# HKU-BAL/Clair

Hardware: AMD Instinct MI355X
Metric: candidate sites/sec (whole node) (higher is better)
Workload: dtype f32 (matmuls as 2-way fp16 split on MFMA with fp32 accumulate; gates/activations fp32); 1 GPU; ONT 122HD34 weights-shape model (random init), synthetic ont-profile pileup tensors, batch=1024, 4 batches in flight per GPU, inputs resident in HBM; batch=1024, streams=4, candidates_total=38912, device_warm_steps=251, collective=none (1 rank), transport=none

## Files before the change

### clair_amd/_capi.py

```python
import ctypes
import os

import numpy as np

from clair_amd._hostapi import Handle

_HERE = os.path.dirname(os.path.abspath(__file__))
LIB_PATH = os.environ.get("CLAIR_AMD_LIB") or os.path.join(_HERE, "libclair_amd.so")

c_int, c_i64, c_vp, c_cp, c_dbl = ctypes.c_int, ctypes.c_int64, ctypes.c_void_p, ctypes.c_char_p, ctypes.c_double
p_vp, p_i64 = ctypes.POINTER(c_vp), ctypes.POINTER(c_i64)


def _sig(*argtypes, **kw):
    return kw.get("restype", c_int), list(argtypes)


_SUBMIT_EX = (c_vp, c_int, c_vp, c_int, c_i64, c_int, c_vp, c_vp, c_vp, c_vp, c_vp, c_vp)
_INFLATE_BLOCKS = (c_vp, c_vp, c_i64, c_int, c_vp, c_vp, c_vp, c_vp, c_vp, c_vp)
SIGNATURES = {
    "clair_abi_version": _sig(),
    "clair_device_count": _sig(),
    "clair_device_pci_bus_id": _sig(c_int, c_cp, c_int),
    "clair_last_error": _sig(c_vp, restype=c_cp),
# ... 380 lines not shown
        mask = int(bool(on))
        if only:
            mask = 0
            for k in only:
                mask |= 1 << KERNEL_NAMES.index(k)
        self._check(self._lib.clair_timing_enable(self._h, mask), "clair_timing_enable")

    def timing_reset(self):
        self._check(self._lib.clair_timing_reset(self._h), "clair_timing_reset")

    def kernel_times(self):
        ms = np.zeros(len(KERNEL_NAMES), dtype=np.float64)
        cnt = np.zeros(len(KERNEL_NAMES), dtype=np.int64)
        self._check(self._lib.clair_kernel_times(self._h, _ptr(ms), _ptr(cnt)), "clair_kernel_times")
        return {k: (float(ms[i]), int(cnt[i])) for i, k in enumerate(KERNEL_NAMES)}

    def kernel_workgroups(self, n):
        wg = np.zeros(len(KERNEL_NAMES), dtype=np.int32)
        self._check(self._lib.clair_kernel_workgroups(self._h, int(n), _ptr(wg)), "clair_kernel_workgroups")
        return {k: int(wg[i]) for i, k in enumerate(KERNEL_NAMES)}

    def counter(self, name):
        v = ctypes.c_int64()
        self._check(self._lib.clair_engine_counter(self._h, ("fused_launches", "fused_recoveries").index(name), ctypes.byref(v)), "clair_engine_counter")
        return int(v.value)

    def debug_read(self, slot, which, shape):
        out = np.empty(shape, dtype=np.float32)
        self._check(self._lib.clair_debug_read(self._h, int(slot), int(which), _ptr(out), out.size), "clair_debug_read")
        return out


class SiteTable(DeviceHandle):

    def __init__(self, engine):
        self._lib = engine._lib
        self._engine = engine
        out = self._own(self._lib.clair_sites_destroy, self._lib.clair_last_error)
        engine._check(self._lib.clair_sites_create(engine._h, out), "clair_sites_create")
        self.n_out = 0

    def _check(self, rc, what):
        if rc != 0:
            raise EngineError("%s failed: %s" % (what, self._last_error(self._engine._h).decode()))

    def begin_source(self, positions):
        p = np.ascontiguousarray(positions, dtype=np.int64)
# ... 390 lines not shown
```

### clair_amd/_hostapi.py

```python
import ctypes
import os

import numpy as np

_HERE = os.path.dirname(os.path.abspath(__file__))
LIB_PATH = os.path.join(_HERE, "libclair_host.so")
vp, cp, i32, i64, f64 = ctypes.c_void_p, ctypes.c_char_p, ctypes.c_int, ctypes.c_int64, ctypes.c_double
p_vp, p_i32, p_i64 = ctypes.POINTER(vp), ctypes.POINTER(i32), ctypes.POINTER(i64)


def _sig(*argtypes, **kw):
    return kw.get("restype", i32), list(argtypes)


_DECODE_ROWS = (vp, vp, vp, vp, vp, cp, vp, i32, i32, i32, i32, i32, i32, vp, i64, p_i64, p_i32)
_FEED = (vp, vp, i64, i32, p_i64)
SIGNATURES = {
    "clair_host_abi_version": _sig(),
    "clair_host_last_error": _sig(restype=cp),
    "clair_host_threads": _sig(i32),
    "clair_host_crc32c": _sig(cp, i64, restype=ctypes.c_uint32),
    "clair_host_counts_to_input_i16": _sig(vp, i64, vp),
    "clair_host_counts_to_input_i32": _sig(vp, i64, vp),
    "clair_host_parse_tensors": _sig(vp, i64, i32, i32, vp, vp, p_i32, p_i32, p_i64),
# ... 41 lines not shown
    "clair_host_bam_render": _sig(vp, vp, vp, i64, i32, i64, i64, p_vp, p_i64),
    "clair_host_faidx": _sig(cp, cp, i64, i64, vp, i64, p_i64),
    "clair_host_bam_set_inflater": _sig(vp, vp, vp, i32),
    "clair_host_inflate_block": _sig(vp, i64, vp, i64, p_i64, ctypes.POINTER(ctypes.c_uint32), p_i32),
    "clair_host_inflate_bgzf": _sig(vp, i64, vp, p_i64, p_i32),
    "clair_host_ensemble_average": _sig(vp, i32, i64, vp),
    "clair_host_ensemble_quantise": _sig(vp, i64, vp),
    "clair_host_ensemble_value": _sig(vp, i64, vp),
    "clair_host_overlap_keep": _sig(vp, i64, vp),
    "clair_host_train_set_key": _sig(cp, i64, i32, p_i64),
    "clair_host_train_set_sample": _sig(vp, i64, vp, i64, f64, f64, i64, vp, vp, vp, p_i64, p_i64),
    "clair_host_train_set_pair_count": _sig(vp, i64, vp, i64, vp, vp, i64, p_i64, p_i64),
    "clair_host_train_set_ratio": _sig(i64, f64, i64, ctypes.POINTER(f64)),
    "clair_host_train_set_pair_keep": _sig(vp, i64, vp, i64, vp, vp, i64, f64, i64, vp, p_i64, p_i64),
    "clair_host_train_set_labels": _sig(vp, vp, i64, vp, vp, i64, vp, vp, i64, vp, vp),
    "clair_host_sites_create": _sig(p_vp),
    "clair_host_sites_destroy": _sig(vp, restype=None),
    "clair_host_sites_begin_source": _sig(vp, vp, i64, p_i64),
    "clair_host_sites_add_rows": _sig(vp, i64, vp, i64, vp, vp, vp),
    "clair_host_sites_finish": _sig(vp, i32, i32, p_i64),
    "clair_host_sites_info": _sig(vp, i64, i64, vp, vp, vp),
    "clair_host_sites_rows": _sig(vp, i64, i64, vp),
    "clair_host_sites_windows": _sig(vp, i64, i64, vp),
}
SYMBOLS = tuple(SIGNATURES)
N_VALUES = 1056
_lib = None


def load():
    global _lib
    if _lib is None:
        if not os.path.isfile(LIB_PATH):
            raise RuntimeError("%s not found: run `python -m clair_amd.build`" % LIB_PATH)
        lib = ctypes.CDLL(LIB_PATH)
        for name, (restype, argtypes) in SIGNATURES.items():
            fn = getattr(lib, name)
            fn.restype, fn.argtypes = restype, argtypes
        if lib.clair_host_abi_version() != 6:
            raise RuntimeError("libclair_host.so has ABI version %d, expected 6: run `python -m clair_amd.build`"
                               % lib.clair_host_abi_version())
        _lib = lib
    return _lib


class Handle(object):
# ... 774 lines not shown
    kv, kn = ctypes.c_int64(0), ctypes.c_int64(0)
    _ts_check(load().clair_host_train_set_pair_keep(p.ctypes.data, len(p), t.ctypes.data, len(t), bs.ctypes.data, be.ctypes.data, nb, float(r), int(key),
                                                    kept.ctypes.data, ctypes.byref(kv), ctypes.byref(kn)))
    return kept[:kv.value + kn.value], kv.value


def train_set_pair(centres, truth, bed, amp, key):
    v, c = train_set_pair_count(centres, truth, bed)
    r = train_set_ratio(v, amp, c)
    kept, kv = train_set_pair_keep(centres, truth, bed, r, key)
    return kept, dict(v=v, c=c, r=r, kept_var=kv, kept_non=len(kept) - kv)


def train_set_labels(centres, centre_base, truth, truth_labels, bed):
    p = np.ascontiguousarray(centres, dtype=np.int64)
    b = np.ascontiguousarray(centre_base, dtype=np.uint8)
    t = np.ascontiguousarray(truth, dtype=np.int64)
    tl = np.ascontiguousarray(truth_labels, dtype=np.uint8).reshape(len(t), 4)
    bs, be, nb = merged_bed(bed)
    labels, in_set = np.zeros((len(p), 4), np.uint8), np.zeros(len(p), np.uint8)
    _ts_check(load().clair_host_train_set_labels(p.ctypes.data, b.ctypes.data, len(p), t.ctypes.data, tl.ctypes.data, len(t), bs.ctypes.data, be.ctypes.data, nb,
                                                 labels.ctypes.data, in_set.ctypes.data))
    return labels, in_set
```

### clair_amd/build.py

```python
import os
import subprocess
import sys

HERE = os.path.dirname(os.path.abspath(__file__))
SRCS = [os.path.join(HERE, "csrc", f) for f in ("engine.hip", "comm.hip", "frontend.hip", "inflate.hip", "overlap.hip", "train.hip")]
OUT = os.path.join(HERE, "libclair_amd.so")
HIPCC = os.environ.get("HIPCC", "/opt/rocm/bin/hipcc")


def csrc_digest(root=None):
    import hashlib
    root = root or os.path.join(HERE, "csrc")
    h = hashlib.sha256()
    for f in sorted(os.listdir(root)):
        if (f.endswith(".hip.h") and not f.startswith("train_")) or f in ("engine.hip", "weight_images.h", "device_buffer.h", "ensemble_core.h"):
            h.update(f.encode() + b"\0" + open(os.path.join(root, f), "rb").read() + b"\0")
    return h.hexdigest()[:16]


def needs_build():
    if not os.path.isfile(OUT):
        return True
    newest = max(os.path.getmtime(os.path.join(dp, f))
                 for dp, _, fs in os.walk(os.path.join(HERE, "csrc")) for f in fs)
    newest = max([newest] + [os.path.getmtime(os.path.join(HERE, "..", "include", h)) for h in ("clair_amd.h", "clair_call.h", "clair_reads.h")])
    return newest > os.path.getmtime(OUT)


HOST_SRCS = [os.path.join(HERE, "hostsrc", f) for f in ("host_io.cpp", "host_decode.cpp", "host_pileup.cpp", "host_sampack.cpp",
                                                              "host_bam.cpp", "host_inflate.cpp", "host_indel.cpp", "host_ensemble.cpp", "host_overlap.cpp", "host_sites.cpp", "host_train_set.cpp")]
HOST_OUT = os.path.join(HERE, "libclair_host.so")
CXX = os.environ.get("CXX", "g++")


def build_host(force=False):
    hdrs = [os.path.join(HERE, "..", "include", h) for h in ("clair_host.h", "clair_reads.h", "clair_call.h", "clair_amd.h")]
    hdrs.append(os.path.join(HERE, "hostsrc", "sam_line.h"))
    hdrs.append(os.path.join(HERE, "csrc", "inflate_core.h"))
    hdrs.append(os.path.join(HERE, "csrc", "indel_lookup_core.h"))
    hdrs.append(os.path.join(HERE, "csrc", "ensemble_core.h"))
    hdrs.append(os.path.join(HERE, "csrc", "overlap_core.h"))
    hdrs.append(os.path.join(HERE, "csrc", "train_set_core.h"))
    if (force or not os.path.isfile(HOST_OUT)
            or max([os.path.getmtime(f) for f in HOST_SRCS + hdrs]) > os.path.getmtime(HOST_OUT)):
        subprocess.check_call([CXX, "-O3", "-std=c++17", "-ffp-contract=off", "-pthread", "-shared", "-fPIC", "-Wall"] + HOST_SRCS + ["-o", HOST_OUT, "-lz"])
    return HOST_OUT


def build(force=False, verbose=False):
    build_host(force)
    if not force and not needs_build():
        return OUT
    cmd = [HIPCC, "--offload-arch=gfx950", "-O3", "-fno-slp-vectorize", "-std=c++17", "-shared", "-fPIC"] + SRCS + ["-o", OUT, "-ldl"]
    if verbose:
        cmd.insert(1, "-Rpass-analysis=kernel-resource-usage")
    subprocess.check_call(cmd)
    return OUT


WAITALL_OUT = os.path.join(HERE, "libclair_amd_waitall.so")


def build_waitall():
    subprocess.check_call([HIPCC, "--offload-arch=gfx950", "-O3", "-fno-slp-vectorize", "-std=c++17", "-shared", "-fPIC", "-DCLAIR_WAIT_ALL"]
                          + SRCS + ["-o", WAITALL_OUT, "-ldl"])
# ... 20 lines not shown
```

### clair_amd/csrc/engine.hip

```cpp
#include "../../include/clair_amd.h"

#include <hip/hip_runtime.h>
#include <ctype.h>

#include <algorithm>
#include <atomic>
#include <cmath>
#include <cstdarg>
#include <cstdio>
#include <cstdlib>
#include <condition_variable>
#include <cstring>
#include <deque>
#include <list>
#include <memory>
#include <mutex>
#include <string>
#include <thread>
#include <vector>

#include "common.hip.h"
#include "dense.hip.h"
#include "decode.hip.h"
#include "evaluate.hip.h"
#include "ensemble.hip.h"
#include "gemm_split.hip.h"
#include "lstm32.hip.h"
#include "lstm32_pair.hip.h"
#include "lstm2_fused.hip.h"
#include "sites.hip.h"
#include "device_buffer.h"
#include "weight_images.h"

using namespace clair;

namespace {

thread_local std::string g_create_error;
thread_local std::string *g_error_sink = nullptr;

constexpr LayerSizes LAYER_SIZES = {T_POS, F_IN, HID, L3_UNITS, L4_UNITS, L5_UNITS, L34_GROUPS, L34_KS, L34_CH, L32_X_SHIFT};

struct TimedLaunch {
    int kernel;
    hipEvent_t start, stop;
};

struct Lane {
    hipStream_t stream = nullptr;
    DeviceBuffer zx;
    DeviceBuffer a1;
    DeviceBuffer a2;
    DeviceBuffer l4part;
    DeviceBuffer fuse_flags;
    unsigned fuse_ticket = 0;
    int last_n_pad = 0;
    std::mutex order;
    std::vector<TimedLaunch> timed;
    std::vector<hipEvent_t> free_events;
    struct FusedRun { const float *x; float *out; int n; int slot; };
    std::vector<FusedRun> fused_runs;
};

struct Slot {
    int lane = 0;
    hipStream_t cin = nullptr, cout = nullptr;
    hipEvent_t ev_in = nullptr, ev_done = nullptr, ev_out = nullptr;
    DeviceBuffer d_x;
    DeviceBuffer d_out;
    PinnedBuffer h_out;
    PinnedBuffer h_x;
    DeviceBuffer d_counts;
    DeviceBuffer d_records;
    PinnedBuffer h_counts;
    DeviceBuffer d_centre; PinnedBuffer h_centre;
    DeviceBuffer d_calls; PinnedBuffer h_calls;
    clair_call_t *o_calls = nullptr;
    DeviceBuffer d_labels; PinnedBuffer h_labels;
    DeviceBuffer d_acc;
    DeviceBuffer d_seq; PinnedBuffer h_seq;
    float *o_gt21 = nullptr, *o_gt = nullptr, *o_l1 = nullptr, *o_l2 = nullptr;
    int pending_n = 0;
    bool refetch = false;
    int staged = 0;
    std::string worker_error;
};

struct ModelWeights {
// ... 20 lines not shown
    int cur = 0;
    int64_t src_n = -1;
    DeviceBuffer pos, lb, is_new, before, row_of;
    DeviceBuffer overflow;
    bool finished = false;
    int64_t n_out = 0;
    DeviceBuffer keep, out_before, out_row, out_key, out_count, out_seq, avg;
    DeviceBuffer gathered;
    SiteRows rows() const { return SiteRows{key.as<int64_t>(), count.as<int>(), acc.as<double>(), x.as<float>(), centre.as<unsigned char>(), seq.as<unsigned char>()}; }
};

struct clair_engine {
    int device = 0;
    int max_batch = 0;
    int max_pad = 0;
    unsigned timing_mask = 0;
    int lstm2_pair = -1;
    std::atomic<int> lstm2_fused{0};
    int fused_groups = 4;
    int64_t fused_launches = 0;
    int64_t fused_fault_at = 0;
    int fused_recoveries = 0;
    int proj2_groups = 8;
    bool l34_stamps = false;
    bool tap_l3 = false;
    std::string error;
    std::list<PinnedBuffer> pinned;
    mutable std::mutex pinned_mu;
    std::vector<Slot> slots;
    std::vector<std::unique_ptr<Lane>> lanes;
    std::vector<hipStream_t> copy_streams;
    int copy_mode = 3;
    bool convert_on_lane = true;
    bool d2h_kernel = true;
    struct Request {
        const void *input; bool counts; int64_t stride; int n;
        const uint8_t *centre; clair_call_t *calls; float *gt21, *gt, *l1, *l2;
        const uint8_t *labels = nullptr;
        int models = 0;
        clair_sites *sites = nullptr;
        int64_t sites_first = 0;
        const uint8_t *seq = nullptr;
    };
    int staging_threads = 2;
    std::vector<std::thread> workers;
    std::mutex wmu;
    std::condition_variable wcv, wdone;
    std::deque<std::pair<int, Request>> wqueue;
    bool wstop = false;
    std::vector<std::unique_ptr<ModelWeights>> models;
    DeviceBuffer eval_counts;
    std::list<std::unique_ptr<clair_sites>> tables;
    double ms_sum[CLAIR_K_COUNT] = {0};
    int64_t launches[CLAIR_K_COUNT] = {0};
};

namespace {

int fail(clair_engine *e, const char *fmt, ...) {
    char buf[512];
    va_list ap;
    va_start(ap, fmt);
    vsnprintf(buf, sizeof buf, fmt, ap);
    va_end(ap);
    if (g_error_sink) *g_error_sink = buf; else if (e) e->error = buf; else g_create_error = buf;
    return 1;
}

#define HIP_TRY(e, call)                                                                        \
    do {                                                                                        \
        hipError_t err__ = (call);                                                              \
        if (err__ != hipSuccess)                                                                \
            return fail((e), "%s failed: %s (%s:%d)", #call, hipGetErrorString(err__), __FILE__, __LINE__); \
    } while (0)

template <typename T> int upload(clair_engine *e, DeviceBuffer &dst, const std::vector<T> &src) {
    dst.reset();
    HIP_TRY(e, dst.ensure(src.size() * sizeof(T)));
    HIP_TRY(e, hipMemcpy(dst.p, src.data(), src.size() * sizeof(T), hipMemcpyHostToDevice));
    return 0;
}

hipEvent_t get_event(Lane &l) {
    if (!l.free_events.empty()) {
        hipEvent_t ev = l.free_events.back();
        l.free_events.pop_back();
        return ev;
    }
    hipEvent_t ev = nullptr;
    (void)hipEventCreate(&ev);
    return ev;
}

struct KernelTimer {
    clair_engine *e; Lane &l; int id; hipEvent_t start = nullptr, stop = nullptr;
    KernelTimer(clair_engine *e_, Lane &l_, int id_) : e(e_), l(l_), id(id_) {
        if ((e->timing_mask >> id) & 1u) { start = get_event(l); stop = get_event(l); (void)hipEventRecord(start, l.stream); }
    }
// ... 10 lines not shown
        Lane &l = *lp;
        HIP_TRY(e, hipStreamSynchronize(l.stream));
        for (auto &t : l.timed) {
            float ms = 0.f;
            HIP_TRY(e, hipEventElapsedTime(&ms, t.start, t.stop));
            e->ms_sum[t.kernel] += ms;
            e->launches[t.kernel] += 1;
            l.free_events.push_back(t.start);
            l.free_events.push_back(t.stop);
        }
        l.timed.clear();
    }
    return 0;
}

bool fused_possible(const clair_engine *e) { return e->lstm2_fused == 1; }
bool use_lstm2_fused(const clair_engine *e, int ntiles) {
    if ((ntiles & 1) || !fused_possible(e)) return false;
    return e->lstm2_fused == 1 || (ntiles >= 16 && ntiles <= 64);
}
size_t fuse_words(int max_pad) { return (size_t)2 * (max_pad / 32) * T_POS * 8; }
size_t fuse_claims(const clair_engine *e) { return (size_t)32 * e->fused_groups + 32 * ((e->max_pad / 64 + 7) / 8); }
bool use_lstm2_pair(const clair_engine *e, int ntiles) { return e->lstm2_pair < 0 ? ntiles >= 64 : e->lstm2_pair == 1; }

int enqueue_forward(clair_engine *e, Lane &l, const ModelWeights &w, const float *x_dev, float *out_dev, int n, int slot_index) {
    const int n_pad = (n + 31) & ~31;
    const int ntiles = n_pad / L32_TILE;
    const int m_rows = T_POS * n_pad;
    l.last_n_pad = n_pad;
    {
        KernelTimer kt(e, l, CLAIR_K_LSTM1);
        Lstm32Args a{x_dev, w.wx1s.as<unsigned short>(), w.bx1.as<float>(), nullptr, w.wh1s.as<unsigned short>(), l.a1.as<unsigned short>(), nullptr, n_pad, ntiles, -1};
        hipLaunchKernelGGL((lstm32_kernel<true>), dim3(ntiles * 2), dim3(256), 0, l.stream, a);
    }
    if (use_lstm2_fused(e, ntiles)) {
        KernelTimer kt(e, l, CLAIR_K_LSTM2);
        const int groups = e->fused_groups;
        if (++l.fuse_ticket == 0) l.fuse_ticket = 1;
        Lstm2FusedArgs a{GemmSplitArgs{l.a1.as<unsigned short>(), w.wx2s.as<unsigned short>(), w.bx2.as<float>(), l.zx.as<float>(), n_pad, ntiles, m_rows, groups},
                         Lstm32Args{nullptr, nullptr, nullptr, l.zx.as<float>(), w.wh2s.as<unsigned short>(), nullptr, l.a2.as<float>(), n_pad, ntiles, -1},
                         FuseArgs{l.fuse_flags.as<unsigned>(), l.fuse_ticket, l.fuse_flags.as<unsigned>() + fuse_words(e->max_pad) + 1, l.fuse_flags.as<unsigned>() + fuse_words(e->max_pad)}, 32 * groups};
        const int consumers = 32 * ((ntiles / 2 + 7) / 8);
        const bool fault = ++e->fused_launches == e->fused_fault_at;
        if (fault) HIP_TRY(e, hipMemsetD32Async((hipDeviceptr_t)a.f.claims, (int)l.fuse_ticket, 1, l.stream));
        hipLaunchKernelGGL(lstm2_fused_kernel, dim3(32 * groups + consumers), dim3(256), 0, l.stream, a);
        if (fault) HIP_TRY(e, hipMemsetAsync(l.a2.as<float>(), 0x7f, (size_t)T_POS * n_pad * 256 * sizeof(float), l.stream));
        l.fused_runs.push_back({x_dev, out_dev, n, slot_index});
    } else {
        {
            KernelTimer kt(e, l, CLAIR_K_PROJ2);
            const int x_tiles = (m_rows + GS_ROWS - 1) / GS_ROWS;
            const int groups = std::min(e->proj2_groups, (x_tiles + 7) / 8);
            GemmSplitArgs a{l.a1.as<unsigned short>(), w.wx2s.as<unsigned short>(), w.bx2.as<float>(), l.zx.as<float>(), n_pad, ntiles, m_rows, groups};
            hipLaunchKernelGGL(gemm_split_kernel, dim3(32 * groups), dim3(256), 0, l.stream, a);
        }
        {
            KernelTimer kt(e, l, CLAIR_K_LSTM2);
            if (use_lstm2_pair(e, ntiles)) {
                Lstm32PairArgs a{l.zx.as<float>(), w.wh2s.as<unsigned short>(), l.a2.as<float>(), n_pad, ntiles};
                hipLaunchKernelGGL(lstm32_pair_kernel, dim3(((ntiles + 1) / 2) * 2), dim3(256), 0, l.stream, a);
            } else {
                Lstm32Args a{nullptr, nullptr, nullptr, l.zx.as<float>(), w.wh2s.as<unsigned short>(), nullptr, l.a2.as<float>(), n_pad, ntiles, -1};
                hipLaunchKernelGGL((lstm32_kernel<false>), dim3(ntiles * 2), dim3(256), 0, l.stream, a);
            }
        }
    }
    {
        KernelTimer kt(e, l, CLAIR_K_L4);
        L3L4Args a{l.a2.as<float>(), w.w3s.as<unsigned short>(), w.w4s.as<unsigned short>(), l.l4part.as<float>(), n_pad, std::ldexp(1.0f, -w.w3_shift), e->tap_l3 ? l.zx.as<float>() : nullptr,
                   e->l34_stamps ? l.zx.as<unsigned long long>() : nullptr};
        hipLaunchKernelGGL(l3l4_kernel, dim3(l34_grid((n_pad + L34_CAND - 1) / L34_CAND)), dim3(L34_THREADS), 0, l.stream, a);
    }
    {
        KernelTimer kt(e, l, CLAIR_K_TAIL);
        TailArgs a{l.l4part.as<float>(), w.b4.as<float>(), w.w5s.as<unsigned short>(), w.b5.as<float>(), w.whs.as<unsigned short>(), w.bh.as<float>(), out_dev, n_pad, n, std::ldexp(1.0f, -w.w4_shift) / L34_ACT_SCALE, {}, {}};
// ... 172 lines not shown
    else if (i - out_vec < call_vec) h_calls[i - out_vec] = calls[i - out_vec];
    if (i == 0 && word) *h_word = *word;
}

int enqueue_results(clair_engine *e, Lane &l, Slot &s, int n, bool calls, bool probs) {
    unsigned *word = l.fuse_flags.p ? l.fuse_flags.as<unsigned>() + fuse_words(e->max_pad) : nullptr;
    unsigned *h_word = (unsigned *)(s.h_out.as<float>() + h_word_offset(e->max_batch));
    if (e->d2h_kernel) {
        const int out_vec = probs ? (n * OUT_FLOATS * (int)sizeof(float) + 15) / 16 : 0, call_vec = calls ? n * (int)sizeof(clair_call_t) / 16 : 0;
        hipLaunchKernelGGL(results_to_host_kernel, dim3((std::max(out_vec + call_vec, 1) + 255) / 256), dim3(256), 0, s.cout, s.d_out.as<uint4>(), s.h_out.as<uint4>(), out_vec,
                           s.d_calls.as<uint4>(), s.h_calls.as<uint4>(), call_vec, word, h_word);
    } else {
        if (calls) HIP_TRY(e, hipMemcpyAsync(s.h_calls.p, s.d_calls.p, (size_t)n * sizeof(clair_call_t), hipMemcpyDeviceToHost, s.cout));
        if (probs) HIP_TRY(e, hipMemcpyAsync(s.h_out.p, s.d_out.p, (size_t)n * OUT_FLOATS * sizeof(float), hipMemcpyDeviceToHost, s.cout));
        if (word) HIP_TRY(e, hipMemcpyAsync(h_word, word, sizeof(unsigned), hipMemcpyDeviceToHost, s.cout));
    }
    HIP_TRY(e, hipEventRecord(s.ev_out, s.cout));
    return 0;
}

int enqueue_request(clair_engine *e, int slot_index, const clair_engine::Request &q) {
    Slot &s = e->slots[slot_index];
    Lane &l = *e->lanes[s.lane];
    const int n = q.n, n_pad = (n + 31) & ~31;
    const bool want_probs = q.gt21 != nullptr;
    const bool same_in = s.cin == l.stream, same_out = s.cout == l.stream;
    std::unique_lock<std::mutex> whole(l.order, std::defer_lock);
    if (same_in) whole.lock();
    const size_t row_bytes = CLAIR_INPUT_FLOATS * (q.counts ? sizeof(short) : sizeof(float));
    const size_t stride = q.stride ? (size_t)q.stride : row_bytes;
    const size_t span = (size_t)(n - 1) * stride + row_bytes;
    const float *own_input;
    { std::lock_guard<std::mutex> g(e->pinned_mu); own_input = s.h_x.as<float>(); }
    const bool direct = (q.input == (const void *)own_input && own_input && stride == row_bytes && !q.counts) || in_pinned(e, q.input, span);
    const bool on_device = !direct && is_device_pointer(q.input);
    if (on_device && !q.counts) return fail(e, "a device pointer is taken for int16 counts only");
    enum { NONE, DENSE, STRIDED } convert = NONE;
    const char *convert_from = nullptr;
    if (q.counts) {
        if (!on_device && ensure_slot_counts(e, s)) return 1;
        if (on_device) {
            convert = STRIDED; convert_from = (const char *)q.input;
        } else if (direct && stride != row_bytes) {
            if (ensure_slot_records(e, s, span, stride)) return 1;
            HIP_TRY(e, hipMemcpyAsync(s.d_records.p, q.input, span, hipMemcpyHostToDevice, s.cin));
            convert = STRIDED; convert_from = s.d_records.as<char>();
// ... 219 lines not shown
    return 0;
}

const char *clair_last_error(const clair_engine_t *e) { return e ? e->error.c_str() : g_create_error.c_str(); }

int clair_engine_create(int device, int max_batch, int n_slots, clair_engine_t **out) {
    if (!out) return fail(nullptr, "out is NULL");
    *out = nullptr;
    if (max_batch < 1 || max_batch > (1 << 20)) return fail(nullptr, "max_batch %d out of range [1, 2^20]", max_batch);
    if (n_slots < 1 || n_slots > 64) return fail(nullptr, "n_slots %d out of range [1,64]", n_slots);
    int ndev = 0;
    hipError_t err = hipGetDeviceCount(&ndev);
    if (err != hipSuccess || ndev <= 0)
        return fail(nullptr, "no HIP device available (hipGetDeviceCount: %s); the MI355X engine has no CPU fallback",
                    hipGetErrorString(err));
    if (device < 0 || device >= ndev) return fail(nullptr, "device %d out of range [0,%d)", device, ndev);
    HIP_TRY(nullptr, hipSetDevice(device));
    clair_engine *e = new clair_engine();
    e->device = device;
    e->max_batch = max_batch;
    e->max_pad = (max_batch + 31) & ~31;
    { const char *t = getenv("CLAIR_AMD_TAP_L3"); e->tap_l3 = t && t[0] == '1'; }
    { const char *t = getenv("CLAIR_AMD_L34_STAMPS"); e->l34_stamps = !e->tap_l3 && t && t[0] == '1'; }
    int n_lanes = n_slots <= 4 ? n_slots : 3;
    { const char *t = getenv("CLAIR_AMD_LANES"); if (t && atoi(t) > 0) n_lanes = std::min(atoi(t), n_slots); }
    e->proj2_groups = n_lanes >= 4 ? 3 : (n_lanes > 1 ? 4 : 8);
    { const char *t = getenv("CLAIR_AMD_PROJ2_GROUPS"); if (t && atoi(t) > 0) e->proj2_groups = atoi(t); }
    { const char *t = getenv("CLAIR_AMD_LSTM2_FUSED"); if (t && (t[0] == '0' || t[0] == '1')) e->lstm2_fused = t[0] - '0'; }
    { const char *t = getenv("CLAIR_AMD_FUSED_GROUPS"); if (t && atoi(t) > 0 && atoi(t) <= 8) e->fused_groups = atoi(t); }
    { const char *t = getenv("CLAIR_AMD_LSTM2_PAIR"); if (t && (t[0] == '0' || t[0] == '1')) e->lstm2_pair = t[0] - '0'; }
    { const char *t = getenv("CLAIR_AMD_FUSED_FAULT"); if (t && atoll(t) > 0) e->fused_fault_at = atoll(t); }
    { const char *t = getenv("CLAIR_AMD_STAGING_THREADS"); if (t && atoi(t) >= 0 && atoi(t) <= 16) e->staging_threads = atoi(t); }
    { const char *t = getenv("CLAIR_AMD_ASYNC_STAGING"); if (t && t[0] == '0') e->staging_threads = 0; }
    { const char *t = getenv("CLAIR_AMD_COPY_STREAMS"); if (t) e->copy_mode = !strcmp(t, "slot") ? 0 : !strcmp(t, "two") ? 1 : !strcmp(t, "lane") ? 2 : 3; }
    { const char *t = getenv("CLAIR_AMD_D2H"); if (t) e->d2h_kernel = !strcmp(t, "kernel"); }
    { const char *t = getenv("CLAIR_AMD_CONVERT"); if (t) e->convert_on_lane = strcmp(t, "copy") != 0; }
    e->models.emplace_back(new ModelWeights());
    for (int i = 0; i < n_lanes; ++i) e->lanes.emplace_back(new Lane());
    e->slots = std::vector<Slot>(n_slots);
    const size_t mp = e->max_pad;
    hipError_t r = hipSuccess;
    for (auto &lp : e->lanes) {
        Lane &l = *lp;
        if (r == hipSuccess) r = hipStreamCreateWithFlags(&l.stream, hipStreamNonBlocking);
        if (r == hipSuccess) r = l.zx.ensure((size_t)T_POS * mp * 1024 * sizeof(float));
        if (r == hipSuccess) r = l.a1.ensure(((size_t)2 * T_POS * mp * 256 + 128 * 256) * sizeof(unsigned short));
        if (r == hipSuccess) r = l.a2.ensure((size_t)T_POS * mp * 256 * sizeof(float));
        if (r == hipSuccess) r = l.l4part.ensure((size_t)L4_SPLITS * ((mp + L34_CAND - 1) / L34_CAND * L34_CAND) * L4_UNITS * sizeof(float));
        if (r == hipSuccess && fused_possible(e)) {
            const size_t words = fuse_words(e->max_pad) + 1 + fuse_claims(e);
            r = l.fuse_flags.ensure(words * sizeof(unsigned));
            if (r == hipSuccess) r = hipMemset(l.fuse_flags.p, 0, words * sizeof(unsigned));
        }
    }
    for (size_t i = 0; i < e->slots.size(); ++i) {
        Slot &s = e->slots[i];
        s.lane = (int)(i % e->lanes.size());
        if (e->copy_mode == 0) {
            hipStream_t st = nullptr;
            if (r == hipSuccess) r = hipStreamCreateWithFlags(&st, hipStreamNonBlocking);
            if (r == hipSuccess) e->copy_streams.push_back(st);
            s.cin = s.cout = st;
        } else if (e->copy_mode == 1) {
            while (r == hipSuccess && e->copy_streams.size() < 2) {
                hipStream_t st = nullptr;
                r = hipStreamCreateWithFlags(&st, hipStreamNonBlocking);
                if (r == hipSuccess) e->copy_streams.push_back(st);
            }
            if (r == hipSuccess) { s.cin = e->copy_streams[0]; s.cout = e->copy_streams[1]; }
        } else if (e->copy_mode == 2) {
            s.cin = s.cout = e->lanes[s.lane]->stream;
        } else {
            if (r == hipSuccess && e->copy_streams.empty()) {
                hipStream_t st = nullptr;
                r = hipStreamCreateWithFlags(&st, hipStreamNonBlocking);
                if (r == hipSuccess) e->copy_streams.push_back(st);
            }
            if (r == hipSuccess) { s.cin = e->copy_streams[0]; s.cout = e->lanes[s.lane]->stream; }
        }
        if (r == hipSuccess) r = hipEventCreateWithFlags(&s.ev_in, hipEventDisableTiming);
// ... 548 lines not shown
    HIP_TRY(e, hipDeviceSynchronize());
    HIP_TRY(e, hipFree(x_dev));
    HIP_TRY(e, hipFree(out_dev));
    return 0;
}

int clair_dataset_upload(clair_engine_t *e, void *x_dev, int64_t first, const float *x_host, int64_t n) {
    if (!e) return fail(nullptr, "engine is NULL");
    HIP_TRY(e, hipSetDevice(e->device));
    HIP_TRY(e, hipMemcpy((float *)x_dev + (size_t)first * CLAIR_INPUT_FLOATS, x_host, (size_t)n * CLAIR_INPUT_FLOATS * sizeof(float), hipMemcpyHostToDevice));
    return 0;
}

int clair_dataset_download(clair_engine_t *e, const void *out_dev, int64_t first, float *out_host, int64_t n) {
    if (!e) return fail(nullptr, "engine is NULL");
    HIP_TRY(e, hipSetDevice(e->device));
    HIP_TRY(e, hipMemcpy(out_host, (const float *)out_dev + (size_t)first * OUT_FLOATS, (size_t)n * OUT_FLOATS * sizeof(float), hipMemcpyDeviceToHost));
    return 0;
}

int clair_run_resident(clair_engine_t *e, int slot, const void *x_dev, void *out_dev, int64_t first, int n) {
    if (check_slot(e, slot) || check_n(e, n)) return 1;
    HIP_TRY(e, hipSetDevice(e->device));
    Lane &l = *e->lanes[e->slots[slot].lane];
    std::lock_guard<std::mutex> g(l.order);
    return enqueue_forward(e, l, *e->models[0], (const float *)x_dev + (size_t)first * CLAIR_INPUT_FLOATS, (float *)out_dev + (size_t)first * OUT_FLOATS, n, -1);
}

int clair_sync(clair_engine_t *e) {
    if (!e) return fail(nullptr, "engine is NULL");
    HIP_TRY(e, hipSetDevice(e->device));
    if (quiesce(e)) return 1;
    return check_fused_placement(e);
}

int clair_timing_enable(clair_engine_t *e, int on) {
    if (!e) return fail(nullptr, "engine is NULL");
    HIP_TRY(e, hipSetDevice(e->device));
    if (drain_timers(e)) return 1;
    e->timing_mask = on == 0 ? 0u : (on == 1 ? ~0u : (unsigned)on);
    return 0;
}

int clair_kernel_times(clair_engine_t *e, double *ms_sum, int64_t *launches) {
    if (!e) return fail(nullptr, "engine is NULL");
    HIP_TRY(e, hipSetDevice(e->device));
    if (drain_timers(e)) return 1;
// ... 1 lines not shown
        if (ms_sum) ms_sum[k] = e->ms_sum[k];
        if (launches) launches[k] = e->launches[k];
    }
    return 0;
}

int clair_timing_reset(clair_engine_t *e) {
    if (!e) return fail(nullptr, "engine is NULL");
    HIP_TRY(e, hipSetDevice(e->device));
    if (drain_timers(e)) return 1;
    for (int k = 0; k < CLAIR_K_COUNT; ++k) { e->ms_sum[k] = 0; e->launches[k] = 0; }
    return 0;
}

int clair_kernel_workgroups(clair_engine_t *e, int n, int *workgroups) {
    if (!e) return fail(nullptr, "engine is NULL");
    if (!workgroups) return fail(e, "workgroups is NULL");
    if (n < 1 || n > e->max_batch) return fail(e, "n %d out of range [1,%d]", n, e->max_batch);
    const int n_pad = (n + 31) & ~31, ntiles = n_pad / 32;
    const int x_tiles = (T_POS * n_pad + GS_ROWS - 1) / GS_ROWS;
    for (int k = 0; k < CLAIR_K_COUNT; ++k) workgroups[k] = 0;
    workgroups[CLAIR_K_LSTM1] = ntiles * 2;
    workgroups[CLAIR_K_LSTM2] = use_lstm2_pair(e, ntiles) ? ((ntiles + 1) / 2) * 2 : ntiles * 2;
    workgroups[CLAIR_K_PROJ2] = 32 * std::min(e->proj2_groups, (x_tiles + 7) / 8);
    if (use_lstm2_fused(e, ntiles)) {
        workgroups[CLAIR_K_LSTM2] = 32 * e->fused_groups + 32 * ((ntiles / 2 + 7) / 8);
        workgroups[CLAIR_K_PROJ2] = 0;
    }
    workgroups[CLAIR_K_L4] = l34_grid((n_pad + L34_CAND - 1) / L34_CAND);
    workgroups[CLAIR_K_TAIL] = n_pad / TAIL_TILE;
    workgroups[CLAIR_K_DECODE] = (n + 3) / 4;
    return 0;
}

int clair_pinned_alloc(clair_engine_t *e, int64_t bytes, void **ptr) {
    if (!e) return fail(nullptr, "engine is NULL");
    if (!ptr || bytes < 1) return fail(e, "bad arguments to clair_pinned_alloc");
    HIP_TRY(e, hipSetDevice(e->device));
    std::list<PinnedBuffer> one(1);
    HIP_TRY(e, one.front().ensure((size_t)bytes));
    *ptr = one.front().p;
    std::lock_guard<std::mutex> g(e->pinned_mu);
    e->pinned.splice(e->pinned.end(), one);
    return 0;
}

int clair_pinned_free(clair_engine_t *e, void *ptr) {
    if (!e) return fail(nullptr, "engine is NULL");
    bool known = false;
    {
        std::lock_guard<std::mutex> g(e->pinned_mu);
        for (const auto &b : e->pinned) known |= b.p == ptr;
    }
    if (!known) return fail(e, "clair_pinned_free: not a buffer of clair_pinned_alloc");
    HIP_TRY(e, hipSetDevice(e->device));
    if (quiesce(e)) return 1;
    std::lock_guard<std::mutex> g(e->pinned_mu);
    e->pinned.remove_if([ptr](const PinnedBuffer &b) { return b.p == ptr; });
    return 0;
}

int clair_engine_counter(clair_engine_t *e, int which, int64_t *value) {
    if (!e) return fail(nullptr, "engine is NULL");
    if (!value) return fail(e, "value is NULL");
    switch (which) {
        case 0: *value = e->fused_launches; return 0;
        case 1: *value = e->fused_recoveries; return 0;
        default: return fail(e, "clair_engine_counter: unknown counter %d", which);
    }
}

int clair_debug_read(clair_engine_t *e, int slot, int which, float *host, int64_t count) {
    if (check_slot(e, slot)) return 1;
    HIP_TRY(e, hipSetDevice(e->device));
    if (quiesce(e)) return 1;
    Lane &l = *e->lanes[e->slots[slot].lane];
    const float *src = nullptr;
    int64_t avail = 0;
    const int64_t np = l.last_n_pad;
    if (which == 1) {
        avail = (int64_t)T_POS * np * 256;
        if (count > avail) return fail(e, "clair_debug_read: asked %lld floats, tap 1 holds %lld", (long long)count, (long long)avail);
        std::vector<unsigned short> planes((size_t)2 * avail);
        HIP_TRY(e, hipMemcpy(planes.data(), l.a1.p, planes.size() * sizeof(unsigned short), hipMemcpyDeviceToHost));
        for (int64_t i = 0; i < count; ++i) host[i] = f16_value(planes[i]) + f16_value(planes[avail + i]);
        return 0;
    }
    if (which == 2) {
        avail = (int64_t)T_POS * np * 256;
        if (count > avail) return fail(e, "clair_debug_read: asked %lld floats, tap 2 holds %lld", (long long)count, (long long)avail);
        std::vector<float> raw((size_t)avail);
        HIP_TRY(e, hipMemcpy(raw.data(), l.a2.p, raw.size() * sizeof(float), hipMemcpyDeviceToHost));
        for (int64_t i = 0; i < count; ++i) {
            const int64_t t = i / (np * 256), n = (i / 256) % np, c = i % 256;
            host[i] = raw[(size_t)((((c / 8) * T_POS + t) * np + n) * 8 + c % 8)];
        }
        return 0;
    }
    switch (which) {
// ... 28 lines not shown
```

### include/clair_host.h

```cpp
#ifndef CLAIR_HOST_H
#define CLAIR_HOST_H
#include <stdint.h>
#include "clair_call.h"
#ifdef __cplusplus
extern "C" {
#endif

#define CLAIR_HOST_ABI_VERSION 6
#define CLAIR_HOST_VALUES 1056

int clair_host_abi_version(void);
const char *clair_host_last_error(void);
int clair_host_threads(int work_items);
uint32_t clair_host_crc32c(const uint8_t *data, int64_t n);

int clair_host_counts_to_input_i16(const int16_t *counts, int64_t n_quads, float *x);
int clair_host_counts_to_input_i32(const int32_t *counts, int64_t n_quads, float *x);

int clair_host_parse_tensors(const char *buf, int64_t len, int final, int max_rows,
                             float *x, int32_t *tok, int *rows_taken, int *rows_kept, int64_t *bytes_consumed);

int clair_host_decode_rows(const float *x, const float *gt21, const float *genotype, const float *len1, const float *len2,
                           const char *meta, const int32_t *meta_tok, int n, int show_reference, int haploid_precision,
                           int haploid_sensitive, int qual_threshold, int arith_numpy2, char *out, int64_t out_cap,
// ... 89 lines not shown
int clair_host_sites_add_rows(clair_host_sites_t *t, int64_t first, const float *probs, int64_t n, const float *x, const uint8_t *centre, const uint8_t *seq);
int clair_host_sites_finish(clair_host_sites_t *t, int min_count, int order, int64_t *n_out);
int clair_host_sites_info(clair_host_sites_t *t, int64_t first, int64_t n, int64_t *positions, int32_t *counts, uint8_t *seq);
int clair_host_sites_rows(clair_host_sites_t *t, int64_t first, int64_t n, float *out);
int clair_host_sites_windows(clair_host_sites_t *t, int64_t first, int64_t n, float *x);

#ifndef CLAIR_OVERLAP_SPAN_T
#define CLAIR_OVERLAP_SPAN_T
typedef struct clair_overlap_span clair_overlap_span_t;
#endif
int clair_host_overlap_keep(const clair_overlap_span_t *spans, int64_t n, uint8_t *keep);

int clair_host_train_set_key(const char *ctg_name, int64_t seed, int stage, int64_t *key);
int clair_host_train_set_sample(const int64_t *positions, int64_t n, const int64_t *truth, int64_t n_truth, double p_near, double p_outside, int64_t key,
                                uint8_t *cls, uint64_t *draws, uint8_t *sampled, int64_t *n_near, int64_t *n_outside);
int clair_host_train_set_pair_count(const int64_t *centres, int64_t n, const int64_t *truth, int64_t n_truth, const int64_t *bed_start, const int64_t *bed_end,
                                    int64_t n_bed, int64_t *v, int64_t *c);
int clair_host_train_set_ratio(int64_t v, double amp, int64_t c, double *r);
int clair_host_train_set_pair_keep(const int64_t *centres, int64_t n, const int64_t *truth, int64_t n_truth, const int64_t *bed_start, const int64_t *bed_end,
                                   int64_t n_bed, double r, int64_t key, int64_t *kept, int64_t *n_kept_var, int64_t *n_kept_non);
int clair_host_train_set_labels(const int64_t *centres, const uint8_t *centre_base, int64_t n, const int64_t *truth, const uint8_t *truth_labels, int64_t n_truth,
                                const int64_t *bed_start, const int64_t *bed_end, int64_t n_bed, uint8_t *labels, uint8_t *in_set);

#ifdef __cplusplus
}
#endif
#endif
```

Baseline: 8.415 million candidates/s.

## Lazily allocate extra resident lanes and round-robin resident batches across HW queues

```diff
diff --git a/clair_amd/_capi.py b/clair_amd/_capi.py
--- a/clair_amd/_capi.py
+++ b/clair_amd/_capi.py
@@ -426,7 +426,7 @@
 
     def counter(self, name):
         v = ctypes.c_int64()
-        self._check(self._lib.clair_engine_counter(self._h, ("fused_launches", "fused_recoveries").index(name), ctypes.byref(v)), "clair_engine_counter")
+        self._check(self._lib.clair_engine_counter(self._h, ("fused_launches", "fused_recoveries", "lanes", "hw_queues").index(name), ctypes.byref(v)), "clair_engine_counter")
         return int(v.value)
 
     def debug_read(self, slot, which, shape):
diff --git a/clair_amd/_hostapi.py b/clair_amd/_hostapi.py
--- a/clair_amd/_hostapi.py
+++ b/clair_amd/_hostapi.py
@@ -87,6 +87,7 @@
     "clair_host_sites_info": _sig(vp, i64, i64, vp, vp, vp),
     "clair_host_sites_rows": _sig(vp, i64, i64, vp),
     "clair_host_sites_windows": _sig(vp, i64, i64, vp),
+    "clair_host_lane_rule": _sig(i32, i32, i32, i32, p_i32, p_i32, p_i32),
 }
 SYMBOLS = tuple(SIGNATURES)
 N_VALUES = 1056
@@ -907,3 +908,10 @@
     _ts_check(load().clair_host_train_set_labels(p.ctypes.data, b.ctypes.data, len(p), t.ctypes.data, tl.ctypes.data, len(t), bs.ctypes.data, be.ctypes.data, nb,
                                                  labels.ctypes.data, in_set.ctypes.data))
     return labels, in_set
+
+
+def lane_rule(n_slots, env_lanes=0, hw_queues=4, fused=False):
+    eager, resident, wanted = i32(), i32(), i32()
+    if load().clair_host_lane_rule(int(n_slots), int(env_lanes), int(hw_queues), int(bool(fused)), ctypes.byref(eager), ctypes.byref(resident), ctypes.byref(wanted)) != 0:
+        raise ValueError(load().clair_host_last_error().decode())
+    return eager.value, resident.value, wanted.value
diff --git a/clair_amd/build.py b/clair_amd/build.py
--- a/clair_amd/build.py
+++ b/clair_amd/build.py
@@ -28,7 +28,7 @@
 
 
 HOST_SRCS = [os.path.join(HERE, "hostsrc", f) for f in ("host_io.cpp", "host_decode.cpp", "host_pileup.cpp", "host_sampack.cpp",
-                                                              "host_bam.cpp", "host_inflate.cpp", "host_indel.cpp", "host_ensemble.cpp", "host_overlap.cpp", "host_sites.cpp", "host_train_set.cpp")]
+                                                              "host_bam.cpp", "host_inflate.cpp", "host_indel.cpp", "host_ensemble.cpp", "host_overlap.cpp", "host_sites.cpp", "host_train_set.cpp", "host_lanes.cpp")]
 HOST_OUT = os.path.join(HERE, "libclair_host.so")
 CXX = os.environ.get("CXX", "g++")
 
@@ -41,6 +41,7 @@
     hdrs.append(os.path.join(HERE, "csrc", "ensemble_core.h"))
     hdrs.append(os.path.join(HERE, "csrc", "overlap_core.h"))
     hdrs.append(os.path.join(HERE, "csrc", "train_set_core.h"))
+    hdrs.append(os.path.join(HERE, "csrc", "lane_rule.h"))
     if (force or not os.path.isfile(HOST_OUT)
             or max([os.path.getmtime(f) for f in HOST_SRCS + hdrs]) > os.path.getmtime(HOST_OUT)):
         subprocess.check_call([CXX, "-O3", "-std=c++17", "-ffp-contract=off", "-pthread", "-shared", "-fPIC", "-Wall"] + HOST_SRCS + ["-o", HOST_OUT, "-lz"])
diff --git a/clair_amd/csrc/engine.hip b/clair_amd/csrc/engine.hip
--- a/clair_amd/csrc/engine.hip
+++ b/clair_amd/csrc/engine.hip
@@ -2,6 +2,8 @@
 
 #include <hip/hip_runtime.h>
 #include <ctype.h>
+#include <dirent.h>
+#include <unistd.h>
 
 #include <algorithm>
 #include <atomic>
@@ -30,6 +32,7 @@
 #include "lstm2_fused.hip.h"
 #include "sites.hip.h"
 #include "device_buffer.h"
+#include "lane_rule.h"
 #include "weight_images.h"
 
 using namespace clair;
@@ -64,6 +67,7 @@
 
 struct Slot {
     int lane = 0;
+    int last_lane = 0;
     hipStream_t cin = nullptr, cout = nullptr;
     hipEvent_t ev_in = nullptr, ev_done = nullptr, ev_out = nullptr;
     DeviceBuffer d_x;
@@ -130,6 +134,7 @@
     int64_t fused_fault_at = 0;
     int fused_recoveries = 0;
     int proj2_groups = 8;
+    int proj2_groups_resident = 8;
     bool l34_stamps = false;
     bool tap_l3 = false;
     std::string error;
@@ -137,6 +142,10 @@
     mutable std::mutex pinned_mu;
     std::vector<Slot> slots;
     std::vector<std::unique_ptr<Lane>> lanes;
+    int eager_lanes = 0;
+    std::mutex resident_mu;
+    int resident_last_slot = -1, resident_last_lane = -1;
+    std::atomic<bool> resident_ready{false};
     std::vector<hipStream_t> copy_streams;
     int copy_mode = 3;
     bool convert_on_lane = true;
@@ -182,6 +191,38 @@
             return fail((e), "%s failed: %s (%s:%d)", #call, hipGetErrorString(err__), __FILE__, __LINE__); \
     } while (0)
 
+int g_hw_queues = HW_QUEUES_MIN;
+bool g_runtime_was_up = false;
+
+bool process_holds_kfd() {
+    DIR *d = opendir("/proc/self/fd");
+    if (!d) return false;
+    bool found = false;
+    while (const dirent *ent = readdir(d)) {
+        char link[64], target[64];
+        snprintf(link, sizeof link, "/proc/self/fd/%s", ent->d_name);
+        const ssize_t len = readlink(link, target, sizeof target - 1);
+        if (len == 8 && !memcmp(target, "/dev/kfd", 8)) { found = true; break; }
+    }
+    closedir(d);
+    return found;
+}
+
+int env_int(const char *name) { const char *t = getenv(name); return t ? atoi(t) : 0; }
+
+__attribute__((constructor)) void ask_for_hw_queues() {
+    g_runtime_was_up = process_holds_kfd();
+    if (g_runtime_was_up) {
+        const int have = env_int("GPU_MAX_HW_QUEUES");
+        g_hw_queues = have > 0 ? std::min(have, HW_QUEUES_MAX) : HW_QUEUES_MIN;
+        return;
+    }
+    g_hw_queues = hw_queues_wanted(env_int("CLAIR_AMD_LANES"));
+    char value[16];
+    snprintf(value, sizeof value, "%d", g_hw_queues);
+    setenv("GPU_MAX_HW_QUEUES", value, 1);
+}
+
 template <typename T> int upload(clair_engine *e, DeviceBuffer &dst, const std::vector<T> &src) {
     dst.reset();
     HIP_TRY(e, dst.ensure(src.size() * sizeof(T)));
@@ -238,6 +279,30 @@
 size_t fuse_words(int max_pad) { return (size_t)2 * (max_pad / 32) * T_POS * 8; }
 size_t fuse_claims(const clair_engine *e) { return (size_t)32 * e->fused_groups + 32 * ((e->max_pad / 64 + 7) / 8); }
 bool use_lstm2_pair(const clair_engine *e, int ntiles) { return e->lstm2_pair < 0 ? ntiles >= 64 : e->lstm2_pair == 1; }
+
+hipError_t allocate_lane(clair_engine *e, Lane &l) {
+    const size_t mp = e->max_pad;
+    hipError_t r = l.zx.ensure((size_t)T_POS * mp * 1024 * sizeof(float));
+    if (r == hipSuccess) r = l.a1.ensure(((size_t)2 * T_POS * mp * 256 + 128 * 256) * sizeof(unsigned short));
+    if (r == hipSuccess) r = l.a2.ensure((size_t)T_POS * mp * 256 * sizeof(float));
+    if (r == hipSuccess) r = l.l4part.ensure((size_t)L4_SPLITS * ((mp + L34_CAND - 1) / L34_CAND * L34_CAND) * L4_UNITS * sizeof(float));
+    if (r == hipSuccess && fused_possible(e)) {
+        const size_t words = fuse_words(e->max_pad) + 1 + fuse_claims(e);
+        r = l.fuse_flags.ensure(words * sizeof(unsigned));
+        if (r == hipSuccess) r = hipMemset(l.fuse_flags.p, 0, words * sizeof(unsigned));
+    }
+    return r;
+}
+
+int ensure_resident_lanes(clair_engine *e) {
+    if (e->resident_ready) return 0;
+    for (size_t i = e->eager_lanes; i < e->lanes.size(); ++i) {
+        const hipError_t r = allocate_lane(e, *e->lanes[i]);
+        if (r != hipSuccess) return fail(e, "allocating the workspaces of lane %d (max_batch=%d) failed: %s", (int)i, e->max_batch, hipGetErrorString(r));
+    }
+    e->resident_ready = true;
+    return 0;
+}
 
 int enqueue_forward(clair_engine *e, Lane &l, const ModelWeights &w, const float *x_dev, float *out_dev, int n, int slot_index) {
     const int n_pad = (n + 31) & ~31;
@@ -266,7 +331,7 @@
         {
             KernelTimer kt(e, l, CLAIR_K_PROJ2);
             const int x_tiles = (m_rows + GS_ROWS - 1) / GS_ROWS;
-            const int groups = std::min(e->proj2_groups, (x_tiles + 7) / 8);
+            const int groups = std::min(slot_index < 0 ? e->proj2_groups_resident : e->proj2_groups, (x_tiles + 7) / 8);
             GemmSplitArgs a{l.a1.as<unsigned short>(), w.wx2s.as<unsigned short>(), w.bx2.as<float>(), l.zx.as<float>(), n_pad, ntiles, m_rows, groups};
             hipLaunchKernelGGL(gemm_split_kernel, dim3(32 * groups), dim3(256), 0, l.stream, a);
         }
@@ -485,6 +550,7 @@
 int enqueue_request(clair_engine *e, int slot_index, const clair_engine::Request &q) {
     Slot &s = e->slots[slot_index];
     Lane &l = *e->lanes[s.lane];
+    s.last_lane = s.lane;
     const int n = q.n, n_pad = (n + 31) & ~31;
     const bool want_probs = q.gt21 != nullptr;
     const bool same_in = s.cin == l.stream, same_out = s.cout == l.stream;
@@ -750,11 +816,12 @@
     e->max_pad = (max_batch + 31) & ~31;
     { const char *t = getenv("CLAIR_AMD_TAP_L3"); e->tap_l3 = t && t[0] == '1'; }
     { const char *t = getenv("CLAIR_AMD_L34_STAMPS"); e->l34_stamps = !e->tap_l3 && t && t[0] == '1'; }
-    int n_lanes = n_slots <= 4 ? n_slots : 3;
-    { const char *t = getenv("CLAIR_AMD_LANES"); if (t && atoi(t) > 0) n_lanes = std::min(atoi(t), n_slots); }
-    e->proj2_groups = n_lanes >= 4 ? 3 : (n_lanes > 1 ? 4 : 8);
-    { const char *t = getenv("CLAIR_AMD_PROJ2_GROUPS"); if (t && atoi(t) > 0) e->proj2_groups = atoi(t); }
     { const char *t = getenv("CLAIR_AMD_LSTM2_FUSED"); if (t && (t[0] == '0' || t[0] == '1')) e->lstm2_fused = t[0] - '0'; }
+    const LaneCounts lanes = lane_rule(n_slots, env_int("CLAIR_AMD_LANES"), g_hw_queues, fused_possible(e));
+    e->eager_lanes = lanes.eager;
+    e->proj2_groups = proj2_groups_for(lanes.eager);
+    e->proj2_groups_resident = proj2_groups_for(lanes.resident);
+    { const char *t = getenv("CLAIR_AMD_PROJ2_GROUPS"); if (t && atoi(t) > 0) e->proj2_groups = e->proj2_groups_resident = atoi(t); }
     { const char *t = getenv("CLAIR_AMD_FUSED_GROUPS"); if (t && atoi(t) > 0 && atoi(t) <= 8) e->fused_groups = atoi(t); }
     { const char *t = getenv("CLAIR_AMD_LSTM2_PAIR"); if (t && (t[0] == '0' || t[0] == '1')) e->lstm2_pair = t[0] - '0'; }
     { const char *t = getenv("CLAIR_AMD_FUSED_FAULT"); if (t && atoll(t) > 0) e->fused_fault_at = atoll(t); }
@@ -764,26 +831,15 @@
     { const char *t = getenv("CLAIR_AMD_D2H"); if (t) e->d2h_kernel = !strcmp(t, "kernel"); }
     { const char *t = getenv("CLAIR_AMD_CONVERT"); if (t) e->convert_on_lane = strcmp(t, "copy") != 0; }
     e->models.emplace_back(new ModelWeights());
-    for (int i = 0; i < n_lanes; ++i) e->lanes.emplace_back(new Lane());
+    for (int i = 0; i < lanes.resident; ++i) e->lanes.emplace_back(new Lane());
     e->slots = std::vector<Slot>(n_slots);
     const size_t mp = e->max_pad;
     hipError_t r = hipSuccess;
-    for (auto &lp : e->lanes) {
-        Lane &l = *lp;
-        if (r == hipSuccess) r = hipStreamCreateWithFlags(&l.stream, hipStreamNonBlocking);
-        if (r == hipSuccess) r = l.zx.ensure((size_t)T_POS * mp * 1024 * sizeof(float));
-        if (r == hipSuccess) r = l.a1.ensure(((size_t)2 * T_POS * mp * 256 + 128 * 256) * sizeof(unsigned short));
-        if (r == hipSuccess) r = l.a2.ensure((size_t)T_POS * mp * 256 * sizeof(float));
-        if (r == hipSuccess) r = l.l4part.ensure((size_t)L4_SPLITS * ((mp + L34_CAND - 1) / L34_CAND * L34_CAND) * L4_UNITS * sizeof(float));
-        if (r == hipSuccess && fused_possible(e)) {
-            const size_t words = fuse_words(e->max_pad) + 1 + fuse_claims(e);
-            r = l.fuse_flags.ensure(words * sizeof(unsigned));
-            if (r == hipSuccess) r = hipMemset(l.fuse_flags.p, 0, words * sizeof(unsigned));
-        }
-    }
+    for (auto &lp : e->lanes) if (r == hipSuccess) r = hipStreamCreateWithFlags(&lp->stream, hipStreamNonBlocking);
+    for (int i = 0; i < e->eager_lanes && r == hipSuccess; ++i) r = allocate_lane(e, *e->lanes[i]);
     for (size_t i = 0; i < e->slots.size(); ++i) {
         Slot &s = e->slots[i];
-        s.lane = (int)(i % e->lanes.size());
+        s.lane = s.last_lane = (int)(i % e->eager_lanes);
         if (e->copy_mode == 0) {
             hipStream_t st = nullptr;
             if (r == hipSuccess) r = hipStreamCreateWithFlags(&st, hipStreamNonBlocking);
@@ -1378,7 +1434,17 @@
 int clair_run_resident(clair_engine_t *e, int slot, const void *x_dev, void *out_dev, int64_t first, int n) {
     if (check_slot(e, slot) || check_n(e, n)) return 1;
     HIP_TRY(e, hipSetDevice(e->device));
-    Lane &l = *e->lanes[e->slots[slot].lane];
+    int lane;
+    {
+        std::lock_guard<std::mutex> g(e->resident_mu);
+        if (ensure_resident_lanes(e)) return 1;
+        if ((int)e->lanes.size() == e->eager_lanes) lane = e->slots[slot].lane;
+        else lane = e->resident_last_lane < 0 ? 0 : (slot == e->resident_last_slot ? e->resident_last_lane : (e->resident_last_lane + 1) % (int)e->lanes.size());
+        e->resident_last_slot = slot;
+        e->resident_last_lane = lane;
+        e->slots[slot].last_lane = lane;
+    }
+    Lane &l = *e->lanes[lane];
     std::lock_guard<std::mutex> g(l.order);
     return enqueue_forward(e, l, *e->models[0], (const float *)x_dev + (size_t)first * CLAIR_INPUT_FLOATS, (float *)out_dev + (size_t)first * OUT_FLOATS, n, -1);
 }
@@ -1426,7 +1492,7 @@
     for (int k = 0; k < CLAIR_K_COUNT; ++k) workgroups[k] = 0;
     workgroups[CLAIR_K_LSTM1] = ntiles * 2;
     workgroups[CLAIR_K_LSTM2] = use_lstm2_pair(e, ntiles) ? ((ntiles + 1) / 2) * 2 : ntiles * 2;
-    workgroups[CLAIR_K_PROJ2] = 32 * std::min(e->proj2_groups, (x_tiles + 7) / 8);
+    workgroups[CLAIR_K_PROJ2] = 32 * std::min(e->resident_ready ? e->proj2_groups_resident : e->proj2_groups, (x_tiles + 7) / 8);
     if (use_lstm2_fused(e, ntiles)) {
         workgroups[CLAIR_K_LSTM2] = 32 * e->fused_groups + 32 * ((ntiles / 2 + 7) / 8);
         workgroups[CLAIR_K_PROJ2] = 0;
@@ -1470,6 +1536,8 @@
     switch (which) {
         case 0: *value = e->fused_launches; return 0;
         case 1: *value = e->fused_recoveries; return 0;
+        case 2: *value = (int64_t)e->lanes.size(); return 0;
+        case 3: *value = g_hw_queues; return 0;
         default: return fail(e, "clair_engine_counter: unknown counter %d", which);
     }
 }
@@ -1478,7 +1546,7 @@
     if (check_slot(e, slot)) return 1;
     HIP_TRY(e, hipSetDevice(e->device));
     if (quiesce(e)) return 1;
-    Lane &l = *e->lanes[e->slots[slot].lane];
+    Lane &l = *e->lanes[e->slots[slot].last_lane];
     const float *src = nullptr;
     int64_t avail = 0;
     const int64_t np = l.last_n_pad;
diff --git a/clair_amd/csrc/lane_rule.h b/clair_amd/csrc/lane_rule.h
--- /dev/null
+++ b/clair_amd/csrc/lane_rule.h
@@ -0,0 +1,32 @@
+#pragma once
+
+#include <algorithm>
+
+namespace clair {
+
+constexpr int HOST_FED_SLOTS = 5;
+constexpr int HW_QUEUES_MIN = 4;
+constexpr int HW_QUEUES_MAX = 32;
+
+struct LaneCounts {
+    int eager;
+    int resident;
+};
+
+inline int hw_queues_wanted(int env_lanes) {
+    return std::min(HW_QUEUES_MAX, std::max(HW_QUEUES_MIN, env_lanes));
+}
+
+inline LaneCounts lane_rule(int n_slots, int env_lanes, int hw_queues, bool fused) {
+    if (n_slots >= HOST_FED_SLOTS || fused || n_slots == 1) {
+        const int lanes = env_lanes > 0 ? std::min(env_lanes, n_slots) : (n_slots >= HOST_FED_SLOTS ? 3 : n_slots);
+        return {lanes, lanes};
+    }
+    const int bound = std::max(HW_QUEUES_MIN, std::min(hw_queues, HW_QUEUES_MAX));
+    const int resident = std::min(env_lanes > 0 ? env_lanes : n_slots, bound);
+    return {std::min(n_slots, resident), resident};
+}
+
+inline int proj2_groups_for(int lanes) { return lanes >= 4 ? 3 : (lanes > 1 ? 4 : 8); }
+
+}
diff --git a/clair_amd/hostsrc/host_lanes.cpp b/clair_amd/hostsrc/host_lanes.cpp
--- /dev/null
+++ b/clair_amd/hostsrc/host_lanes.cpp
@@ -0,0 +1,17 @@
+#include "../../include/clair_host.h"
+#include "../csrc/lane_rule.h"
+
+int clair_host_fail(const char *fmt, ...);
+
+extern "C" {
+
+int clair_host_lane_rule(int n_slots, int env_lanes, int hw_queues, int fused, int *eager, int *resident, int *queues_wanted) {
+    if (n_slots < 1 || n_slots > 64 || !eager || !resident || !queues_wanted) return clair_host_fail("lane rule: bad arguments");
+    const clair::LaneCounts c = clair::lane_rule(n_slots, env_lanes, hw_queues, fused != 0);
+    *eager = c.eager;
+    *resident = c.resident;
+    *queues_wanted = clair::hw_queues_wanted(env_lanes);
+    return 0;
+}
+
+}
diff --git a/include/clair_host.h b/include/clair_host.h
--- a/include/clair_host.h
+++ b/include/clair_host.h
@@ -135,6 +135,8 @@
 int clair_host_train_set_labels(const int64_t *centres, const uint8_t *centre_base, int64_t n, const int64_t *truth, const uint8_t *truth_labels, int64_t n_truth,
                                 const int64_t *bed_start, const int64_t *bed_end, int64_t n_bed, uint8_t *labels, uint8_t *in_set);
 
+int clair_host_lane_rule(int n_slots, int env_lanes, int hw_queues, int fused, int *eager, int *resident, int *queues_wanted);
+
 #ifdef __cplusplus
 }
 #endif
```

Measured after the change: 8.010 million candidates/s. 4.8% lower.
